# h33p/ofps

Hardware: AMD Instinct MI355X
Metric: Mvectors/s, 1080p 16x16 blocks +-16 full-search SAD (higher is better)
Workload: dtype u8

## Files before the change

ofps_amd/csrc/sad.hip:

```cpp
#include "common.hpp"

#include <cstdlib>
#include <utility>

namespace {

constexpr int kWavesPerWG = 4;

constexpr int pick_stride(int min_s, int k, int ng) {
    for (int s = min_s; s < min_s + 64; ++s)
        if ((k * s) % 32 == ng % 32) return s;
    return min_s | 1;
}

template <int B, int R, int K>
struct SadCfg {
    static_assert(B % 4 == 0 && R % 4 == 0, "tile origin must stay dword aligned");
    static_assert(B * B * 255 <= 65535, "packed u16 SAD accumulators would overflow");
    static constexpr int NCAND = 2 * R + 1;
    static constexpr int NG = (NCAND + 3) / 4;
    static constexpr int NC = (NCAND + K - 1) / K;
    static constexpr int T = NG * NC;
    static constexpr int PASSES = (T + 63) / 64;
    static constexpr int BW = B / 4;
    static constexpr int TILE_H = B + 2 * R;
    static constexpr int TILE_ROWS = NC * K + B - 1;
    static constexpr int TILE_WD = (kWavesPerWG * B + 2 * R) / 4;
    static constexpr int MAXCOL = (kWavesPerWG - 1) * BW + (NG - 1) + BW;
    static constexpr int MIN_S = (MAXCOL + 1 > TILE_WD) ? MAXCOL + 1 : TILE_WD;
    static constexpr int S = pick_stride(MIN_S, K, NG);
    static constexpr int LDS_DWORDS = TILE_ROWS * S;
};

__device__ __forceinline__ unsigned long long shfl_xor_u64(unsigned long long v, int mask) {
    unsigned lo = (unsigned)v, hi = (unsigned)(v >> 32);
    lo = __shfl_xor(lo, mask, 64);
    hi = __shfl_xor(hi, mask, 64);
    return ((unsigned long long)hi << 32) | lo;
}

struct __attribute__((packed, aligned(4))) U64A4 { unsigned long long v; };

struct SadParams {
    const uint8_t* prev_base;
    const uint8_t* cur_base;
    size_t prev_pitch, cur_pitch;
    int W, H, stride;
    int nbx, nby;
    float nx, ny;
    float4* out_entries;
    int* out_best;
    unsigned long long div_spp, div_spr;
};
inline unsigned long long div_magic48(unsigned d) { return ((1ull << 48) + d - 1) / d; }
__device__ __forceinline__ unsigned div48(unsigned n, unsigned long long m) { return (unsigned)(((unsigned long long)n * m) >> 48); }

__device__ __forceinline__ void write_block_result(const SadParams& p, int pair, int bx, int by, int B, int R,
                                                   unsigned long long key) {
    const int sad = (int)(key >> 48);
    const int dy = (int)((key >> 8) & 0xFF) - R;
    const int dx = (int)(key & 0xFF) - R;
    const size_t k = ((size_t)pair * p.nby + by) * p.nbx + bx;
    const float cx = (float)(bx * B + B / 2 + dx), cy = (float)(by * B + B / 2 + dy);
    float4 e;
    e.x = cx * p.nx;
    e.y = cy * p.ny;
    e.z = ((float)dx / 1.0f) * (-p.nx);
    e.w = ((float)dy / 1.0f) * (-p.ny);
    p.out_entries[k] = e;
    if (p.out_best) {
        p.out_best[3 * k + 0] = dx;
        p.out_best[3 * k + 1] = dy;
        p.out_best[3 * k + 2] = sad;
    }
}

template <int B, int R, int K>
__global__ __launch_bounds__(256) void sad_qsad_kernel(const SadParams p) {
    using C = SadCfg<B, R, K>;
    __shared__ uint32_t tile[C::LDS_DWORDS];

    const int pair = blockIdx.z;
    const uint8_t* __restrict__ prev = p.prev_base + (size_t)pair * p.prev_pitch;
    const uint8_t* __restrict__ cur = p.cur_base + (size_t)pair * p.cur_pitch;
    const int by = blockIdx.y;
    const int bx0 = blockIdx.x * kWavesPerWG;
    const int tid = threadIdx.x;

    const int wave = __builtin_amdgcn_readfirstlane(tid >> 6);
    const int lane = tid & 63;
    const int bx = bx0 + wave;
    const int x0 = bx * B, y0 = by * B;

    uint32_t c[B][C::BW];
    {
        const int bxc = bx < p.nbx ? bx : p.nbx - 1;
        const uint32_t* __restrict__ cp = reinterpret_cast<const uint32_t*>(cur + (size_t)y0 * p.stride + bxc * B);
        const int sdw = p.stride >> 2;
#pragma unroll
        for (int y = 0; y < B; ++y)
#pragma unroll
            for (int q = 0; q < C::BW; ++q) c[y][q] = cp[y * sdw + q];
    }

    {
        const int tx0 = bx0 * B - R, ty0 = by * B - R;
        for (int idx = tid; idx < C::TILE_H * C::TILE_WD; idx += 256) {
            const int row = idx / C::TILE_WD, col = idx - row * C::TILE_WD;
            const int gx = tx0 + 4 * col, gy = ty0 + row;
            if (gy >= 0 && gy < p.H && gx >= 0 && gx < p.W)
                tile[row * C::S + col] = *reinterpret_cast<const uint32_t*>(prev + (size_t)gy * p.stride + gx);
        }
    }
    __syncthreads();
    if (bx >= p.nbx) return;

    unsigned long long best = ~0ull;
#pragma unroll 1
    for (int pass = 0; pass < C::PASSES; ++pass) {
        const int t = pass * 64 + lane;
        const bool active = t < C::T;
        const int tc = active ? t : 0;
        const int chunk = tc / C::NG, g = tc - chunk * C::NG;
        const int dx0 = -R + 4 * g, dy0 = -R + K * chunk;

        unsigned long long acc[K];
#pragma unroll
        for (int i = 0; i < K; ++i) acc[i] = 0;

        const uint32_t* trow = tile + (K * chunk) * C::S + wave * C::BW + g;
#pragma unroll
        for (int rr = 0; rr < B + K - 1; ++rr) {
            unsigned long long win[C::BW];
#pragma unroll
            for (int q = 0; q < C::BW; ++q) win[q] = reinterpret_cast<const U64A4*>(trow + rr * C::S + q)->v;
#pragma unroll
            for (int i = 0; i < K; ++i) {
                const int y = rr - i;
                if (y >= 0 && y < B) {
#pragma unroll
                    for (int q = 0; q < C::BW; ++q) acc[i] = __builtin_amdgcn_qsad_pk_u16_u8(win[q], c[y][q], acc[i]);
                }
            }
        }
        __builtin_amdgcn_sched_group_barrier(0x100, C::BW, 0);
#pragma unroll
        for (int rr = 0; rr < B + K - 1; ++rr) {
            __builtin_amdgcn_sched_group_barrier(0x100, C::BW, 0);
            __builtin_amdgcn_sched_group_barrier(0x002, K * C::BW, 0);
        }

#pragma unroll
        for (int i = 0; i < K; ++i) asm volatile("" : "+v"(acc[i]));

        uint32_t bkey = 0xFFFFFFFFu;
        int bci = 0;
#pragma unroll
        for (int i = 0; i < K; ++i) {
            const int dy = dy0 + i;
            const int vy = (int)active & (int)(dy <= R) & (int)(y0 + dy >= 0) & (int)(y0 + dy + B <= p.H);
#pragma unroll
            for (int j = 0; j < 4; ++j) {
                const int dx = dx0 + j;
                const int v = vy & (int)(dx <= R) & (int)(x0 + dx >= 0) & (int)(x0 + dx + B <= p.W);
                const uint32_t d2inv = (uint32_t)(dx * dx + dy * dy) | (uint32_t)(v - 1);
                const uint32_t half = (j < 2) ? (uint32_t)acc[i] : (uint32_t)(acc[i] >> 32);
                const uint32_t key = ((j & 1) ? (half & 0xFFFF0000u) : (half << 16)) | d2inv;
                const bool lt = key < bkey;
                bkey = lt ? key : bkey;
                bci = lt ? (i * 4 + j) : bci;
            }
        }
        if (bkey != 0xFFFFFFFFu) {
            const int bi = bci >> 2, bj = bci & 3;
            const unsigned long long k64 =
                ((unsigned long long)bkey << 32) | (uint32_t)(((dy0 + bi + R) << 8) | (dx0 + bj + R));
            best = k64 < best ? k64 : best;
        }
    }

#pragma unroll
    for (int m = 32; m >= 1; m >>= 1) {
        const unsigned long long o = shfl_xor_u64(best, m);
        best = o < best ? o : best;
    }
    if (lane == 0) write_block_result(p, pair, bx, by, B, R, best);
}

template <int B, int R>
struct StripCfg {
    static_assert(B % 4 == 0 && R % 4 == 0, "tile origin and the dx = +R column must stay dword aligned");
    static_assert(B * B * 255 <= 65535, "packed u16 SAD accumulators would overflow");
    static constexpr int NCAND = 2 * R + 1;
    static constexpr int NGA = (2 * R) / 4;
    static constexpr int pow2_ceil(int v) { int p = 1; while (p < v) p <<= 1; return p; }
    static constexpr int NG = pow2_ceil(NGA);
    static_assert(NGA >= 1 && NG <= 64, "search range too wide for one wave per strip");
    static constexpr int NB = 64 / NG;
    static constexpr int BW = B / 4;
    static constexpr int TILE_H = B + 2 * R;
    static constexpr int KE = (NCAND + NG - 1) / NG;
    static constexpr int EDGE_COL = (2 * R) / 4;
    static constexpr int GRAN = ((NB * B) % 16 == 0 && R % 16 == 0) ? 16 : (((NB * B) % 8 == 0 && R % 8 == 0) ? 8 : 4);
    static constexpr int GDW = GRAN / 4;
    static constexpr int TILE_WG = (NB * B + 2 * R + GRAN - 1) / GRAN;
    static constexpr int MAXCOL = (NB - 1) * BW + (NG - 1) + BW;
    static constexpr int SW = ((MAXCOL + 1 > TILE_WG * GDW ? MAXCOL + 1 : TILE_WG * GDW) + 3) / 4 * 4;
    static_assert((NB - 1) * BW + EDGE_COL + BW <= SW, "edge column must lie inside a window row");
    static constexpr int TILE_ROWS = TILE_H > NG * KE + B - 1 ? TILE_H : NG * KE + B - 1;
    static constexpr int TILE_DWORDS = TILE_ROWS * SW;
    static_assert(2 * R * R < 65536, "lane key holds d2 in 16 bits");
    static constexpr int SPLIT = (NCAND + 32) / 33;
    static constexpr int NP = (NCAND + SPLIT - 1) / SPLIT;
    static constexpr int MIN_WAVES = (2 * NP + B * BW + 40 <= 168) ? 3 : 2;
    static constexpr bool COMPACT_KEY = ((2 * R * R) << 6) + NCAND < 65536 && NCAND <= 64;
    static constexpr bool RANK_KEY = !COMPACT_KEY && ((2 * R * R) << 3) + 7 < 65536;
    static constexpr int KSHIFT = COMPACT_KEY ? 6 : (RANK_KEY ? 3 : 0);
};

template <int B, int R>
struct StripWalk {
    static constexpr int ROWS_PER_BASE = (255 - StripCfg<B, R>::BW) / StripCfg<B, R>::SW + 1;
};

template <int B, int R, int I0, int RR>
__device__ __forceinline__ void strip_row(unsigned long long (&acc)[StripCfg<B, R>::NP], const uint32_t (&c)[B][B / 4],
                                          const uint32_t* lds, uint32_t& base) {
    using C = StripCfg<B, R>;
    constexpr int G = StripWalk<B, R>::ROWS_PER_BASE;
    if constexpr (RR > 0 && RR % G == 0) {
        base += G * C::SW;
        asm volatile("" : "+v"(base));
    }
    unsigned long long win[C::BW];
#pragma unroll
    for (int q = 0; q < C::BW; ++q) win[q] = reinterpret_cast<const U64A4*>(lds + base + (RR % G) * C::SW + q)->v;
#pragma unroll
    for (int ii = 0; ii < C::NP; ++ii) {
        const int y = RR - ii;
        if (I0 + ii < C::NCAND && y >= 0 && y < B) {
#pragma unroll
            for (int q = 0; q < C::BW; ++q) acc[ii] = __builtin_amdgcn_qsad_pk_u16_u8(win[q], c[y][q], acc[ii]);
        }
    }
}

template <int B, int R, int I0, int... RR>
__device__ __forceinline__ void strip_rows(unsigned long long (&acc)[StripCfg<B, R>::NP], const uint32_t (&c)[B][B / 4],
                                           const uint32_t* lds, uint32_t tile_off, std::integer_sequence<int, RR...>) {
    uint32_t base = tile_off + I0 * StripCfg<B, R>::SW;
    asm volatile("" : "+v"(base));
    (strip_row<B, R, I0, RR>(acc, c, lds, base), ...);
}

#ifndef OFPS_SAD_COLKEYS
#define OFPS_SAD_COLKEYS 2
#endif
constexpr int kSadColKeys = OFPS_SAD_COLKEYS;
constexpr int kColSlotDwords = kSadColKeys == 2 ? 4 * 64 : 0;

template <int B, int R, int I0>
__device__ __forceinline__ void strip_pass(const uint32_t (&c)[B][B / 4], const uint32_t* lds, uint32_t tile_off,
                                           const uint32_t (&colk)[4], const uint32_t (&colk_pos)[4], int y0, int H, uint32_t& bkey, int& bi,
                                           uint32_t (&colmin)[4], uint32_t* amin) {
    using C = StripCfg<B, R>;
    unsigned long long acc[C::NP];
#pragma unroll
    for (int ii = 0; ii < C::NP; ++ii) acc[ii] = 0;
    constexpr int ROWS = ((I0 + C::NP < C::NCAND ? C::NP : C::NCAND - I0) + B - 1);
    strip_rows<B, R, I0>(acc, c, lds, tile_off, std::make_integer_sequence<int, ROWS>{});
#pragma unroll
    for (int ii = 0; ii < C::NP; ++ii) asm volatile("" : "+v"(acc[ii]));
    if constexpr (kSadColKeys != 0 && (C::RANK_KEY || C::COMPACT_KEY)) {
        auto low_of = [&](int ii) -> uint32_t {
            const int i = I0 + ii, dy = -R + i;
            const bool ok = i < C::NCAND && y0 + dy >= 0 && y0 + dy + B <= H;
            return ok ? (uint32_t)(C::RANK_KEY ? ((dy * dy) << 1 | (dy > 0 ? 1 : 0)) : ((dy * dy) << 6 | i)) : 0xFFFFFFFFu;
        };
        uint32_t hmask = 0xFFFF0000u;
        asm volatile("" : "+v"(hmask));
        auto keys_of = [&](int ii, uint32_t low, uint32_t (&k)[4]) {
            const uint32_t lo = (uint32_t)acc[ii], hi = (uint32_t)(acc[ii] >> 32);
            k[0] = (lo << 16) | low; k[1] = (lo & hmask) | low; k[2] = (hi << 16) | low; k[3] = (hi & hmask) | low;
        };
        if constexpr (kSadColKeys == 1) {
#pragma unroll
            for (int ii = 0; ii < C::NP; ii += 2) {
                if (I0 + ii >= C::NCAND) break;
                uint32_t ka[4], kb[4];
                keys_of(ii, low_of(ii), ka);
                if (ii + 1 < C::NP && I0 + ii + 1 < C::NCAND) {
                    keys_of(ii + 1, low_of(ii + 1), kb);
#pragma unroll
                    for (int j = 0; j < 4; ++j)
                        asm("v_min3_u32 %0, %1, %2, %3" : "=v"(colmin[j]) : "v"(colmin[j]), "v"(ka[j]), "v"(kb[j]));
                } else {
#pragma unroll
                    for (int j = 0; j < 4; ++j) colmin[j] = min(colmin[j], ka[j]);
                }
            }
        } else {
#pragma unroll
            for (int ii = 0; ii < C::NP; ++ii) {
                if (I0 + ii >= C::NCAND) break;
                uint32_t k[4];
                keys_of(ii, low_of(ii), k);
#pragma unroll
                for (int j = 0; j < 4; ++j) __hip_atomic_fetch_min(amin + 64 * j, k[j], __ATOMIC_RELAXED, __HIP_MEMORY_SCOPE_WAVEFRONT);
            }
        }
        return;
    }
#pragma unroll
    for (int ii = 0; ii < C::NP; ++ii) {
        const int i = I0 + ii;
        const int dy = -R + i;
        if (i < C::NCAND && y0 + dy >= 0 && y0 + dy + B <= H) {
            const uint32_t lo = (uint32_t)acc[ii], hi = (uint32_t)(acc[ii] >> 32);
            const uint32_t (&ck)[4] = (C::RANK_KEY && dy > 0) ? colk_pos : colk;
            const uint32_t k0 = (lo << 16) | ck[0];
            const uint32_t k1 = (lo & 0xFFFF0000u) | ck[1];
            const uint32_t k2 = (hi << 16) | ck[2];
            const uint32_t k3 = (hi & 0xFFFF0000u) | ck[3];
            if constexpr (C::RANK_KEY) {
                bkey = min(bkey, __builtin_elementwise_add_sat(min(min(k0, k1), min(k2, k3)), (uint32_t)((dy * dy) << 3)));
            } else if constexpr (C::COMPACT_KEY) {
                const uint32_t m = __builtin_elementwise_add_sat(min(min(k0, k1), min(k2, k3)), (uint32_t)((dy * dy) << 6 | i));
                bkey = min(bkey, m);
            } else {
                const uint32_t m = __builtin_elementwise_add_sat(min(min(k0, k1), min(k2, k3)), (uint32_t)(dy * dy));
                const bool lt = m < bkey;
                bkey = lt ? m : bkey;
                bi = lt ? i : bi;
            }
        }
    }
}

template <int B, int R, int... S>
__device__ __forceinline__ void strip_passes(const uint32_t (&c)[B][B / 4], const uint32_t* lds, uint32_t tile_off,
                                             const uint32_t (&colk)[4], const uint32_t (&colk_pos)[4], int y0, int H, uint32_t& bkey, int& bi,
                                             uint32_t (&colmin)[4], uint32_t* amin, std::integer_sequence<int, S...>) {
    (strip_pass<B, R, S * StripCfg<B, R>::NP>(c, lds, tile_off, colk, colk_pos, y0, H, bkey, bi, colmin, amin), ...);
}

constexpr int kStripWaves = 4;

template <int B, int R>
__device__ __forceinline__ void strip_body(const SadParams& p, int strips_per_row, int strip, uint32_t* tiles, int wave, int lane) {
    using C = StripCfg<B, R>;
    const int strips_per_pair = strips_per_row * p.nby;
    const int pair = (int)div48((unsigned)strip, p.div_spp);
    const int rem = strip - pair * strips_per_pair;
    const int by = (int)div48((unsigned)rem, p.div_spr);
    const int bx0 = (rem - by * strips_per_row) * C::NB;

    const uint8_t* __restrict__ prev = p.prev_base + (size_t)pair * p.prev_pitch;
    const uint8_t* __restrict__ cur = p.cur_base + (size_t)pair * p.cur_pitch;
    uint32_t* tile = tiles + wave * C::TILE_DWORDS;

    const int b = lane / C::NG;
    const int g = lane % C::NG;
    const int bx = bx0 + b;
    const bool blk_on = bx < p.nbx;
    const int y0 = by * B;

    uint32_t c[B][C::BW];
    {
        const int bxc = blk_on ? bx : p.nbx - 1;
        const uint8_t* cp = cur + (size_t)y0 * p.stride + bxc * B;
#pragma unroll
        for (int y = 0; y < B; ++y) {
            if constexpr (C::BW % 4 == 0) {
#pragma unroll
                for (int q4 = 0; q4 < C::BW; q4 += 4) {
                    const uint4 v = *reinterpret_cast<const uint4*>(cp + (size_t)y * p.stride + 4 * q4);
                    c[y][q4 + 0] = v.x; c[y][q4 + 1] = v.y; c[y][q4 + 2] = v.z; c[y][q4 + 3] = v.w;
                }
            } else {
#pragma unroll
                for (int q2 = 0; q2 < C::BW; q2 += 2) {
                    const uint2 v = *reinterpret_cast<const uint2*>(cp + (size_t)y * p.stride + 4 * q2);
                    c[y][q2 + 0] = v.x; c[y][q2 + 1] = v.y;
                }
            }
        }
    }

    {
        constexpr int LR = 64 / C::TILE_WG;
        constexpr int STEPS = (C::TILE_H + LR - 1) / LR;
        const int tx0 = bx0 * B - R, ty0 = y0 - R;
        const int sr = lane / C::TILE_WG, sc = lane - sr * C::TILE_WG;
        const int gx = tx0 + C::GRAN * sc;
        const bool lane_on = sr < LR && gx >= 0 && gx < p.W;
        const uint8_t* src = prev + (ptrdiff_t)(ty0 + sr) * p.stride + gx;
        uint32_t* dst = tile + sr * C::SW + C::GDW * sc;
#pragma unroll
        for (int it = 0; it < STEPS; ++it) {
            const int row = sr + it * LR;
            const bool row_in_tile = (it + 1) * LR <= C::TILE_H || row < C::TILE_H;
            if (lane_on && row_in_tile && (unsigned)(ty0 + row) < (unsigned)p.H) {
                const uint8_t* sp = src + (ptrdiff_t)(it * LR) * p.stride;
                uint32_t* dp = dst + it * LR * C::SW;
                if constexpr (C::GRAN == 16) *reinterpret_cast<uint4*>(dp) = *reinterpret_cast<const uint4*>(sp);
                else if constexpr (C::GRAN == 8) *reinterpret_cast<uint2*>(dp) = *reinterpret_cast<const uint2*>(sp);
                else *dp = *reinterpret_cast<const uint32_t*>(sp);
            }
        }
    }
    __builtin_amdgcn_fence(__ATOMIC_RELEASE, "wavefront");
    __builtin_amdgcn_wave_barrier();
    __builtin_amdgcn_fence(__ATOMIC_ACQUIRE, "wavefront");

    const int dx0 = -R + 4 * g;
    uint32_t colk[4], colk_pos[4];
#pragma unroll
    for (int j = 0; j < 4; ++j) {
        const int dx = dx0 + j;
        const int x = bx * B + dx;
        const bool v = blk_on && g < C::NGA && x >= 0 && x + B <= p.W;
        const uint32_t rank = dx0 < 0 ? 3u - j : (uint32_t)j;
        colk[j] = v ? ((uint32_t)(dx * dx) << C::KSHIFT) | (C::RANK_KEY ? rank : 0u) : 0xFFFFFFFFu;
        colk_pos[j] = v ? ((uint32_t)(dx * dx) << C::KSHIFT) | (7u - rank) : 0xFFFFFFFFu;
    }
    uint32_t bkey = 0xFFFFFFFFu;
    int bi = 0;
    uint32_t colmin[4] = {0xFFFFFFFFu, 0xFFFFFFFFu, 0xFFFFFFFFu, 0xFFFFFFFFu};
    uint32_t* amin = nullptr;
    if constexpr (kSadColKeys == 2 && (C::RANK_KEY || C::COMPACT_KEY)) {
        amin = tiles + kStripWaves * C::TILE_DWORDS + wave * kColSlotDwords + lane;
#pragma unroll
        for (int j = 0; j < 4; ++j) amin[64 * j] = 0xFFFFFFFFu;
    }
    strip_passes<B, R>(c, tiles, (uint32_t)(wave * C::TILE_DWORDS + b * C::BW + g), colk, colk_pos, y0, p.H, bkey, bi, colmin, amin,
                       std::make_integer_sequence<int, C::SPLIT>{});
    if constexpr (kSadColKeys != 0 && (C::RANK_KEY || C::COMPACT_KEY)) {
#pragma unroll
        for (int j = 0; j < 4; ++j) {
            uint32_t kc;
            if constexpr (kSadColKeys == 2) kc = __hip_atomic_load(amin + 64 * j, __ATOMIC_RELAXED, __HIP_MEMORY_SCOPE_WAVEFRONT);
            else kc = colmin[j];
            uint32_t lk;
            if constexpr (C::RANK_KEY) {
                const uint32_t x = (((kc & 0xFFFEu) << 2) + colk[j]) ^ ((kc & 1u) * 7u);
                lk = (kc & 0xFFFF0000u) | x;
            } else {
                lk = (kc & 0xFFFF0000u) | ((kc & 0xFFFFu) + colk[j]);
            }
            lk = (colk[j] == 0xFFFFFFFFu || kc == 0xFFFFFFFFu) ? 0xFFFFFFFFu : lk;
            bkey = min(bkey, lk);
        }
    }
    unsigned long long best = ~0ull;
    if (bkey != 0xFFFFFFFFu) {
        const uint32_t d2 = (bkey & 0xFFFFu) >> C::KSHIFT;
        int dx = dx0, dy;
        if constexpr (C::RANK_KEY) {
            const int code = (int)(bkey & 7u);
            const bool neg = code < 4;
            const int rank = neg ? code : 7 - code;
            dx = dx0 + (dx0 < 0 ? 3 - rank : rank);
            const int ady = (int)(__builtin_sqrtf((float)((int)d2 - dx * dx)) + 0.5f);
            dy = neg ? -ady : ady;
        } else {
            if constexpr (C::COMPACT_KEY) bi = (int)(bkey & 63u);
            dy = -R + bi;
            const int dxsq = (int)d2 - dy * dy;
#pragma unroll
            for (int j = 1; j < 4; ++j) dx = ((dx0 + j) * (dx0 + j) == dxsq) ? dx0 + j : dx;
        }
        best = ((unsigned long long)((bkey & 0xFFFF0000u) | d2) << 32) | (unsigned long long)(uint32_t)(((dy + R) << 8) | (dx + R));
    }
    uint32_t eacc[C::KE];
#pragma unroll
    for (int i = 0; i < C::KE; ++i) eacc[i] = 0;
    {
        const uint32_t* ecol = tile + b * C::BW + C::EDGE_COL;
        const int erow0 = g * C::KE;
        uint32_t nxt[C::BW];
#pragma unroll
        for (int q = 0; q < C::BW; ++q) nxt[q] = ecol[erow0 * C::SW + q];
#pragma unroll
        for (int rr = 0; rr < B + C::KE - 1; ++rr) {
            uint32_t ref[C::BW];
#pragma unroll
            for (int q = 0; q < C::BW; ++q) ref[q] = nxt[q];
            if (rr + 1 < B + C::KE - 1) {
                const int row = erow0 + rr + 1;
#pragma unroll
                for (int q = 0; q < C::BW; ++q) nxt[q] = ecol[row * C::SW + q];
            }
#pragma unroll
            for (int i = 0; i < C::KE; ++i) {
                const int y = rr - i;
                if (y >= 0 && y < B) {
#pragma unroll
                    for (int q = 0; q < C::BW; ++q) eacc[i] = __builtin_amdgcn_sad_u8(ref[q], c[y][q], eacc[i]);
                }
            }
            asm volatile("" : "+v"(eacc[0]) : : "memory");
        }
    }

    {
        const bool xok = blk_on && bx * B + R + B <= p.W;
#pragma unroll
        for (int i = 0; i < C::KE; ++i) {
            const int dy = -R + g * C::KE + i;
            const bool v = xok && dy <= R && y0 + dy >= 0 && y0 + dy + B <= p.H;
            const unsigned long long k64 =
                ((unsigned long long)((eacc[i] << 16) | (uint32_t)(R * R + dy * dy)) << 32) |
                (unsigned long long)(uint32_t)(((dy + R) << 8) | (2 * R));
            best = (v && k64 < best) ? k64 : best;
        }
    }
#pragma unroll
    for (int m = 1; m < C::NG; m <<= 1) {
        const unsigned long long o = shfl_xor_u64(best, m);
        best = o < best ? o : best;
    }
    if (blk_on && g == 0) {
        const int sad = (int)(best >> 48);
        const int dy = (int)((best >> 8) & 0xFF) - R, dx = (int)(best & 0xFF) - R;
        const size_t k = ((size_t)pair * p.nby + by) * p.nbx + bx;
        float4 e;
        e.x = (float)(bx * B + B / 2 + dx) * p.nx;
        e.y = (float)(y0 + B / 2 + dy) * p.ny;
        e.z = ((float)dx / 1.0f) * (-p.nx);
        e.w = ((float)dy / 1.0f) * (-p.ny);
        p.out_entries[k] = e;
        if (p.out_best) {
            p.out_best[3 * k + 0] = dx;
            p.out_best[3 * k + 1] = dy;
            p.out_best[3 * k + 2] = sad;
        }
    }
}

template <int B, int R>
__global__ __launch_bounds__(64 * kStripWaves, (StripCfg<B, R>::MIN_WAVES)) void sad_strip_kernel(const SadParams p, int strips_per_row,
                                                                      int total_strips) {
    using C = StripCfg<B, R>;
    __shared__ __attribute__((aligned(16))) uint32_t tiles[kStripWaves * (C::TILE_DWORDS + kColSlotDwords)];
    const int wave = __builtin_amdgcn_readfirstlane(threadIdx.x >> 6);
    const int lane = threadIdx.x & 63;
    const int per_xcd = gridDim.x / 8;
    const int lwg = (int)(blockIdx.x % 8) * per_xcd + (int)(blockIdx.x / 8);
    const int strip = lwg * kStripWaves + wave;
    if (strip >= total_strips) return;
    strip_body<B, R>(p, strips_per_row, strip, tiles, wave, lane);
}

template <int B, int R>
__global__ __launch_bounds__(64 * kStripWaves, (StripCfg<B, R>::MIN_WAVES)) void sad_strip_list_kernel(const SadParams p, int strips_per_row,
                                                                           const uint32_t* __restrict__ strip_list) {
    using C = StripCfg<B, R>;
    __shared__ __attribute__((aligned(16))) uint32_t tiles[kStripWaves * (C::TILE_DWORDS + kColSlotDwords)];
    const int wave = __builtin_amdgcn_readfirstlane(threadIdx.x >> 6);
    const int lane = threadIdx.x & 63;
    const int count = (int)strip_list[0];
#pragma unroll 1
    for (int k = (int)blockIdx.x * kStripWaves + wave; k < count; k += (int)gridDim.x * kStripWaves)
        strip_body<B, R>(p, strips_per_row, (int)strip_list[1 + k], tiles, wave, lane);
}

struct PdeCfg {
    static constexpr int B = 16, R = 16, STEP = 4, PR = B / STEP;
    using C = StripCfg<B, R>;
    static constexpr int CUR_DW = B * C::NB * C::BW;
    static constexpr int CAP = 512;
    static constexpr int WAVE_DW = C::TILE_DWORDS + 4 + CUR_DW + CAP + 2 * C::NB;
    static constexpr int OFF_CUR = C::TILE_DWORDS + 4, OFF_LIST = OFF_CUR + CUR_DW, OFF_BEST = OFF_LIST + CAP;
    static_assert(OFF_BEST % 2 == 0, "64-bit keys must be 8-byte aligned");
};

template <int RR>
__device__ __forceinline__ void pde_row(unsigned long long (&acc)[PdeCfg::C::NP], const uint32_t (&c)[PdeCfg::PR][PdeCfg::C::BW],
                                        const uint32_t* lds, uint32_t& base) {
    using C = PdeCfg::C;
    constexpr int B = PdeCfg::B, R = PdeCfg::R, STEP = PdeCfg::STEP;
    constexpr int G = StripWalk<B, R>::ROWS_PER_BASE;
    if constexpr (RR > 0 && RR % G == 0) {
        base += G * C::SW;
        asm volatile("" : "+v"(base));
    }
    unsigned long long win[C::BW];
#pragma unroll
    for (int q = 0; q < C::BW; ++q) win[q] = reinterpret_cast<const U64A4*>(lds + base + (RR % G) * C::SW + q)->v;
#pragma unroll
    for (int ii = 0; ii < C::NP; ++ii) {
        const int y = RR - ii;
        if (ii < C::NCAND && y >= 0 && y < B && y % STEP == 0) {
#pragma unroll
            for (int q = 0; q < C::BW; ++q) acc[ii] = __builtin_amdgcn_qsad_pk_u16_u8(win[q], c[y / STEP][q], acc[ii]);
        }
    }
}
template <int... RR>
__device__ __forceinline__ void pde_rows(unsigned long long (&acc)[PdeCfg::C::NP], const uint32_t (&c)[PdeCfg::PR][PdeCfg::C::BW],
                                         const uint32_t* lds, uint32_t tile_off, std::integer_sequence<int, RR...>) {
    uint32_t base = tile_off;
    asm volatile("" : "+v"(base));
    (pde_row<RR>(acc, c, lds, base), ...);
}

__device__ __forceinline__ uint32_t pde_two_rows(const uint32_t* tile, const uint32_t* curl, int bb, int dyi, int dxi, int r8) {
    using C = PdeCfg::C;
    const int sh = dxi & 3;
    uint32_t s = 0;
#pragma unroll
    for (int k = 0; k < 2; ++k) {
        const int y = 2 * r8 + k;
        const uint32_t* rp = tile + (dyi + y) * C::SW + bb * C::BW + (dxi >> 2);
        const uint32_t* cp = curl + y * (C::NB * C::BW) + bb * C::BW;
        uint32_t d[C::BW + 1];
#pragma unroll
        for (int q = 0; q <= C::BW; ++q) d[q] = rp[q];
#pragma unroll
        for (int q = 0; q < C::BW; ++q) s = __builtin_amdgcn_sad_u8(__builtin_amdgcn_alignbyte(d[q + 1], d[q], sh), cp[q], s);
    }
    return s;
}

__global__ __launch_bounds__(64 * kStripWaves, 3) void sad_pde_kernel(const SadParams p, int strips_per_row, int total_strips,
                                                                       uint32_t* __restrict__ strip_list) {
    using P = PdeCfg;
    using C = P::C;
    constexpr int B = P::B, R = P::R;
    __shared__ __attribute__((aligned(16))) uint32_t lds[kStripWaves * P::WAVE_DW];

    const int wave = __builtin_amdgcn_readfirstlane(threadIdx.x >> 6);
    const int lane = threadIdx.x & 63;
    const int per_xcd = gridDim.x / 8;
    const int lwg = (int)(blockIdx.x % 8) * per_xcd + (int)(blockIdx.x / 8);
    const int strip = lwg * kStripWaves + wave;
    if (strip >= total_strips) return;
    const int strips_per_pair = strips_per_row * p.nby;
    const int pair = strip / strips_per_pair;
    const int rem = strip - pair * strips_per_pair;
    const int by = rem / strips_per_row;
    const int bx0 = (rem - by * strips_per_row) * C::NB;
    const uint8_t* __restrict__ prev = p.prev_base + (size_t)pair * p.prev_pitch;
    const uint8_t* __restrict__ cur = p.cur_base + (size_t)pair * p.cur_pitch;
    uint32_t* tile = lds + wave * P::WAVE_DW;
    uint32_t* curl = tile + P::OFF_CUR;
    uint32_t* list = tile + P::OFF_LIST;
    unsigned long long* bestk = reinterpret_cast<unsigned long long*>(tile + P::OFF_BEST);

    const int b = lane / C::NG, g = lane % C::NG;
    const int bx = bx0 + b;
    const bool blk_on = bx < p.nbx;
    const int y0 = by * B;

    {
        const int tx0 = bx0 * B - R, ty0 = y0 - R;
        for (int idx = lane; idx < C::TILE_H * C::TILE_WG; idx += 64) {
            const int row = idx / C::TILE_WG, col = idx - row * C::TILE_WG;
            const int gx = tx0 + 16 * col, gy = ty0 + row;
            if (gy >= 0 && gy < p.H && gx >= 0 && gx < p.W)
                *reinterpret_cast<uint4*>(tile + row * C::SW + 4 * col) = *reinterpret_cast<const uint4*>(prev + (size_t)gy * p.stride + gx);
        }
#pragma unroll
        for (int k = 0; k < 2; ++k) {
            const int idx = lane + 64 * k, row = idx / C::NB, blk = idx % C::NB;
            const int bxc = min(bx0 + blk, p.nbx - 1);
            *reinterpret_cast<uint4*>(curl + row * (C::NB * C::BW) + blk * C::BW) =
                *reinterpret_cast<const uint4*>(cur + (size_t)(y0 + row) * p.stride + bxc * B);
        }
    }
    __builtin_amdgcn_fence(__ATOMIC_RELEASE, "wavefront");
    __builtin_amdgcn_wave_barrier();
    __builtin_amdgcn_fence(__ATOMIC_ACQUIRE, "wavefront");

    uint32_t c4[P::PR][C::BW];
#pragma unroll
    for (int r = 0; r < P::PR; ++r)
#pragma unroll
        for (int q = 0; q < C::BW; ++q) c4[r][q] = curl[(P::STEP * r) * (C::NB * C::BW) + b * C::BW + q];
    unsigned long long acc[C::NP];
#pragma unroll
    for (int ii = 0; ii < C::NP; ++ii) acc[ii] = 0;
    pde_rows(acc, c4, lds, (uint32_t)(wave * P::WAVE_DW + b * C::BW + g), std::make_integer_sequence<int, C::NCAND + B - 1>{});
#pragma unroll
    for (int ii = 0; ii < C::NP; ++ii) asm volatile("" : "+v"(acc[ii]));

    const int dx0 = -R + 4 * g;
    bool colv[4];
    uint32_t colk[4];
#pragma unroll
    for (int j = 0; j < 4; ++j) {
        const int x = bx * B + dx0 + j;
        colv[j] = blk_on && x >= 0 && x + B <= p.W;
        colk[j] = colv[j] ? (uint32_t)((dx0 + j) * (dx0 + j)) << C::KSHIFT : 0xFFFFFFFFu;
    }
    static_assert(C::COMPACT_KEY && C::SPLIT == 1, "written for the +-16 geometry");
    uint32_t bkey = 0xFFFFFFFFu;
#pragma unroll
    for (int i = 0; i < C::NCAND; ++i) {
        const int dy = -R + i;
        if (y0 + dy >= 0 && y0 + dy + B <= p.H) {
            const uint32_t lo = (uint32_t)acc[i], hi = (uint32_t)(acc[i] >> 32);
            const uint32_t k0 = (lo << 16) | colk[0], k1 = (lo & 0xFFFF0000u) | colk[1];
            const uint32_t k2 = (hi << 16) | colk[2], k3 = (hi & 0xFFFF0000u) | colk[3];
            bkey = min(bkey, __builtin_elementwise_add_sat(min(min(k0, k1), min(k2, k3)), (uint32_t)((dy * dy) << 6 | i)));
        }
    }
    unsigned long long pbest = ~0ull;
    if (bkey != 0xFFFFFFFFu) {
        const int bi = (int)(bkey & 63u), dy = -R + bi;
        const uint32_t d2 = (bkey & 0xFFFFu) >> C::KSHIFT;
        const int dxsq = (int)d2 - dy * dy;
        int dx = dx0;
#pragma unroll
        for (int j = 1; j < 4; ++j) dx = ((dx0 + j) * (dx0 + j) == dxsq) ? dx0 + j : dx;
        pbest = ((unsigned long long)((bkey & 0xFFFF0000u) | d2) << 32) | (unsigned long long)(uint32_t)(((dy + R) << 8) | (dx + R));
    }
    uint32_t eacc[C::KE];
    const bool xok = blk_on && bx * B + R + B <= p.W;
    {
        const uint32_t* ecol = tile + b * C::BW + C::EDGE_COL;
#pragma unroll
        for (int i = 0; i < C::KE; ++i) {
            const int dyi = min(g * C::KE + i, C::NCAND - 1);
            uint32_t sacc = 0;
#pragma unroll
            for (int r = 0; r < P::PR; ++r)
#pragma unroll
                for (int q = 0; q < C::BW; ++q) sacc = __builtin_amdgcn_sad_u8(ecol[(dyi + P::STEP * r) * C::SW + q], c4[r][q], sacc);
            eacc[i] = sacc;
            const int dy = -R + g * C::KE + i;
            const bool v = xok && dy <= R && y0 + dy >= 0 && y0 + dy + B <= p.H;
            const unsigned long long k64 = ((unsigned long long)((sacc << 16) | (uint32_t)(R * R + dy * dy)) << 32) |
                                           (unsigned long long)(uint32_t)(((dy + R) << 8) | (2 * R));
            pbest = (v && k64 < pbest) ? k64 : pbest;
        }
    }
#pragma unroll
    for (int m = 1; m < C::NG; m <<= 1) {
        const unsigned long long o = shfl_xor_u64(pbest, m);
        pbest = o < pbest ? o : pbest;
    }
    const int dy0i = blk_on ? (int)((pbest >> 8) & 0xFF) : R, dx0i = blk_on ? (int)(pbest & 0xFF) : R;
    auto key64 = [&](uint32_t sad, int dyi, int dxi) {
        const int dy = dyi - R, dx = dxi - R;
        return ((unsigned long long)((sad << 16) | (uint32_t)(dx * dx + dy * dy)) << 32) | (unsigned long long)(uint32_t)((dyi << 8) | dxi);
    };
    uint32_t U = pde_two_rows(tile, curl, b, dy0i, dx0i, g);
#pragma unroll
    for (int m = 1; m < C::NG; m <<= 1) U += __shfl_xor(U, m, 64);
    if (g == 0) bestk[b] = blk_on ? key64(U, dy0i, dx0i) : ~0ull;
    int nlist = 0;
    {
        int uj[4];
#pragma unroll
        for (int j = 0; j < 4; ++j) uj[j] = colv[j] ? (int)U : -1;
        const unsigned long long below = (1ull << lane) - 1ull;
        typedef unsigned short us2 __attribute__((ext_vector_type(2)));
        const uint32_t u1 = min(U + 1u, 0xFFFFu) * 0x10001u;
        auto any_le = [&](uint32_t v) {
            const us2 m = __builtin_elementwise_min(__builtin_bit_cast(us2, v), __builtin_bit_cast(us2, u1));
            return __builtin_bit_cast(uint32_t, m) ^ u1;
        };
#pragma unroll
        for (int i = 0; i < C::NCAND; ++i) {
            const int dy = -R + i;
            if (y0 + dy >= 0 && y0 + dy + B <= p.H) {
                const uint32_t lo = (uint32_t)acc[i], hi = (uint32_t)(acc[i] >> 32);
                if (!__ballot((any_le(lo) | any_le(hi)) != 0u)) continue;
                const int s4[4] = {(int)(lo & 0xFFFFu), (int)(lo >> 16), (int)(hi & 0xFFFFu), (int)(hi >> 16)};
#pragma unroll
                for (int j = 0; j < 4; ++j) {
                    const bool hit = s4[j] <= uj[j];
                    const unsigned long long mask = __ballot(hit);
                    if (mask) {
                        const int pos = nlist + __popcll(mask & below);
                        if (hit && pos < P::CAP) list[pos] = ((uint32_t)b << 16) | ((uint32_t)i << 8) | (uint32_t)(4 * g + j);
                        nlist += __popcll(mask);
                    }
                }
            }
        }
#pragma unroll
        for (int i = 0; i < C::KE; ++i) {
            const int dyi = g * C::KE + i, dy = dyi - R;
            const bool hit = xok && dy <= R && y0 + dy >= 0 && y0 + dy + B <= p.H && eacc[i] <= U;
            const unsigned long long mask = __ballot(hit);
            if (mask) {
                const int pos = nlist + __popcll(mask & below);
                if (hit && pos < P::CAP) list[pos] = ((uint32_t)b << 16) | ((uint32_t)dyi << 8) | (uint32_t)(2 * R);
                nlist += __popcll(mask);
            }
        }
    }
    __builtin_amdgcn_fence(__ATOMIC_RELEASE, "wavefront");
    __builtin_amdgcn_wave_barrier();
    __builtin_amdgcn_fence(__ATOMIC_ACQUIRE, "wavefront");
    const int n = nlist;
    if (n > P::CAP) {
        if (lane == 0) {
            const uint32_t pos = atomicAdd(&strip_list[0], 1u);
            strip_list[1 + pos] = (uint32_t)strip;
        }
        return;
    }
    constexpr int PER_STEP = 2 * (64 / C::NG);
    for (int base = 0; base < n; base += PER_STEP) {
        const int idx0 = base + lane / C::NG, idx1 = idx0 + 64 / C::NG;
        const uint32_t e0 = list[min(idx0, n - 1)], e1 = list[min(idx1, n - 1)];
        const int bb0 = (int)(e0 >> 16), dyi0 = (int)((e0 >> 8) & 0xFF), dxi0 = (int)(e0 & 0xFF);
        const int bb1 = (int)(e1 >> 16), dyi1 = (int)((e1 >> 8) & 0xFF), dxi1 = (int)(e1 & 0xFF);
        uint32_t s0 = pde_two_rows(tile, curl, bb0, dyi0, dxi0, g);
        uint32_t s1 = pde_two_rows(tile, curl, bb1, dyi1, dxi1, g);
#pragma unroll
        for (int m = 1; m < C::NG; m <<= 1) { s0 += __shfl_xor(s0, m, 64); s1 += __shfl_xor(s1, m, 64); }
        if (g == 0 && idx0 < n) atomicMin(&bestk[bb0], key64(s0, dyi0, dxi0));
        if (g == 0 && idx1 < n) atomicMin(&bestk[bb1], key64(s1, dyi1, dxi1));
    }
// ... 296 lines not shown
```

Before: 516.6.

## Clip vertical candidate rows at frame edges and split edge-column SAD work

At blocks near the top or bottom frame edges, a clipped strip path runs only the 8-row candidate chunks that overlap the valid dy range, skipping SAD work for out-of-frame displacements. The dx=+R edge column now spreads 2R rows across lanes. The last dy=+R candidate is computed by a cross-lane partial sum over block rows, using current-block rows loaded straight from global memory. This also raises the minimum-waves hint for the 8x8/R=8 config. The cost is more code paths, extra global loads and a shuffle reduction.

```diff
diff --git a/ofps_amd/csrc/sad.hip b/ofps_amd/csrc/sad.hip
--- a/ofps_amd/csrc/sad.hip
+++ b/ofps_amd/csrc/sad.hip
@@ -200,6 +200,8 @@
     static constexpr int BW = B / 4;
     static constexpr int TILE_H = B + 2 * R;
     static constexpr int KE = (NCAND + NG - 1) / NG;
+    static constexpr int KE2 = (2 * R + NG - 1) / NG;
+    static constexpr int ERL = (B + NG - 1) / NG;
     static constexpr int EDGE_COL = (2 * R) / 4;
     static constexpr int GRAN = ((NB * B) % 16 == 0 && R % 16 == 0) ? 16 : (((NB * B) % 8 == 0 && R % 8 == 0) ? 8 : 4);
     static constexpr int GDW = GRAN / 4;
@@ -212,7 +214,7 @@
     static_assert(2 * R * R < 65536, "lane key holds d2 in 16 bits");
     static constexpr int SPLIT = (NCAND + 32) / 33;
     static constexpr int NP = (NCAND + SPLIT - 1) / SPLIT;
-    static constexpr int MIN_WAVES = (2 * NP + B * BW + 40 <= 168) ? 3 : 2;
+    static constexpr int MIN_WAVES = (B == 8 && R == 8) ? 8 : ((2 * NP + B * BW + 40 <= 168) ? 3 : 2);
     static constexpr bool COMPACT_KEY = ((2 * R * R) << 6) + NCAND < 65536 && NCAND <= 64;
     static constexpr bool RANK_KEY = !COMPACT_KEY && ((2 * R * R) << 3) + 7 < 65536;
     static constexpr int KSHIFT = COMPACT_KEY ? 6 : (RANK_KEY ? 3 : 0);
@@ -223,8 +225,8 @@
     static constexpr int ROWS_PER_BASE = (255 - StripCfg<B, R>::BW) / StripCfg<B, R>::SW + 1;
 };
 
-template <int B, int R, int I0, int RR>
-__device__ __forceinline__ void strip_row(unsigned long long (&acc)[StripCfg<B, R>::NP], const uint32_t (&c)[B][B / 4],
+template <int B, int R, int I0, int N, int RR>
+__device__ __forceinline__ void strip_row(unsigned long long (&acc)[N], const uint32_t (&c)[B][B / 4],
                                           const uint32_t* lds, uint32_t& base) {
     using C = StripCfg<B, R>;
     constexpr int G = StripWalk<B, R>::ROWS_PER_BASE;
@@ -236,7 +238,7 @@
 #pragma unroll
     for (int q = 0; q < C::BW; ++q) win[q] = reinterpret_cast<const U64A4*>(lds + base + (RR % G) * C::SW + q)->v;
 #pragma unroll
-    for (int ii = 0; ii < C::NP; ++ii) {
+    for (int ii = 0; ii < N; ++ii) {
         const int y = RR - ii;
         if (I0 + ii < C::NCAND && y >= 0 && y < B) {
 #pragma unroll
@@ -245,12 +247,12 @@
     }
 }
 
-template <int B, int R, int I0, int... RR>
-__device__ __forceinline__ void strip_rows(unsigned long long (&acc)[StripCfg<B, R>::NP], const uint32_t (&c)[B][B / 4],
+template <int B, int R, int I0, int N, int... RR>
+__device__ __forceinline__ void strip_rows(unsigned long long (&acc)[N], const uint32_t (&c)[B][B / 4],
                                            const uint32_t* lds, uint32_t tile_off, std::integer_sequence<int, RR...>) {
     uint32_t base = tile_off + I0 * StripCfg<B, R>::SW;
     asm volatile("" : "+v"(base));
-    (strip_row<B, R, I0, RR>(acc, c, lds, base), ...);
+    (strip_row<B, R, I0, N, RR>(acc, c, lds, base), ...);
 }
 
 #ifndef OFPS_SAD_COLKEYS
@@ -259,18 +261,18 @@
 constexpr int kSadColKeys = OFPS_SAD_COLKEYS;
 constexpr int kColSlotDwords = kSadColKeys == 2 ? 4 * 64 : 0;
 
-template <int B, int R, int I0>
+template <int B, int R, int I0, int N = StripCfg<B, R>::NP>
 __device__ __forceinline__ void strip_pass(const uint32_t (&c)[B][B / 4], const uint32_t* lds, uint32_t tile_off,
                                            const uint32_t (&colk)[4], const uint32_t (&colk_pos)[4], int y0, int H, uint32_t& bkey, int& bi,
                                            uint32_t (&colmin)[4], uint32_t* amin) {
     using C = StripCfg<B, R>;
-    unsigned long long acc[C::NP];
-#pragma unroll
-    for (int ii = 0; ii < C::NP; ++ii) acc[ii] = 0;
-    constexpr int ROWS = ((I0 + C::NP < C::NCAND ? C::NP : C::NCAND - I0) + B - 1);
-    strip_rows<B, R, I0>(acc, c, lds, tile_off, std::make_integer_sequence<int, ROWS>{});
-#pragma unroll
-    for (int ii = 0; ii < C::NP; ++ii) asm volatile("" : "+v"(acc[ii]));
+    unsigned long long acc[N];
+#pragma unroll
+    for (int ii = 0; ii < N; ++ii) acc[ii] = 0;
+    constexpr int ROWS = ((I0 + N < C::NCAND ? N : C::NCAND - I0) + B - 1);
+    strip_rows<B, R, I0, N>(acc, c, lds, tile_off, std::make_integer_sequence<int, ROWS>{});
+#pragma unroll
+    for (int ii = 0; ii < N; ++ii) asm volatile("" : "+v"(acc[ii]));
     if constexpr (kSadColKeys != 0 && (C::RANK_KEY || C::COMPACT_KEY)) {
         auto low_of = [&](int ii) -> uint32_t {
             const int i = I0 + ii, dy = -R + i;
@@ -285,11 +287,11 @@
         };
         if constexpr (kSadColKeys == 1) {
 #pragma unroll
-            for (int ii = 0; ii < C::NP; ii += 2) {
+            for (int ii = 0; ii < N; ii += 2) {
                 if (I0 + ii >= C::NCAND) break;
                 uint32_t ka[4], kb[4];
                 keys_of(ii, low_of(ii), ka);
-                if (ii + 1 < C::NP && I0 + ii + 1 < C::NCAND) {
+                if (ii + 1 < N && I0 + ii + 1 < C::NCAND) {
                     keys_of(ii + 1, low_of(ii + 1), kb);
 #pragma unroll
                     for (int j = 0; j < 4; ++j)
@@ -301,7 +303,7 @@
             }
         } else {
 #pragma unroll
-            for (int ii = 0; ii < C::NP; ++ii) {
+            for (int ii = 0; ii < N; ++ii) {
                 if (I0 + ii >= C::NCAND) break;
                 uint32_t k[4];
                 keys_of(ii, low_of(ii), k);
@@ -312,7 +314,7 @@
         return;
     }
 #pragma unroll
-    for (int ii = 0; ii < C::NP; ++ii) {
+    for (int ii = 0; ii < N; ++ii) {
         const int i = I0 + ii;
         const int dy = -R + i;
         if (i < C::NCAND && y0 + dy >= 0 && y0 + dy + B <= H) {
@@ -344,6 +346,24 @@
     (strip_pass<B, R, S * StripCfg<B, R>::NP>(c, lds, tile_off, colk, colk_pos, y0, H, bkey, bi, colmin, amin), ...);
 }
 
+template <int B, int R>
+struct StripClip {
+    static constexpr int NCH = (2 * R) / 8 > 0 ? (2 * R) / 8 : 1;
+    static constexpr int start(int k) { return k >= NCH ? StripCfg<B, R>::NCAND : (8 * k > R ? 8 * k + 1 : 8 * k); }
+};
+
+template <int B, int R, int... K>
+__device__ __forceinline__ void strip_clipped(const uint32_t (&c)[B][B / 4], const uint32_t* lds, uint32_t tile_off,
+                                              const uint32_t (&colk)[4], const uint32_t (&colk_pos)[4], int y0, int H, int ilo, int ihi,
+                                              uint32_t& bkey, int& bi, uint32_t (&colmin)[4], uint32_t* amin, std::integer_sequence<int, K...>) {
+    using L = StripClip<B, R>;
+    auto chunk = [&](auto k) {
+        constexpr int S = L::start(decltype(k)::value), E = L::start(decltype(k)::value + 1);
+        if (ihi >= S && ilo < E) strip_pass<B, R, S, E - S>(c, lds, tile_off, colk, colk_pos, y0, H, bkey, bi, colmin, amin);
+    };
+    (chunk(std::integral_constant<int, K>{}), ...);
+}
+
 constexpr int kStripWaves = 4;
 
 template <int B, int R>
@@ -433,8 +453,14 @@
 #pragma unroll
         for (int j = 0; j < 4; ++j) amin[64 * j] = 0xFFFFFFFFu;
     }
-    strip_passes<B, R>(c, tiles, (uint32_t)(wave * C::TILE_DWORDS + b * C::BW + g), colk, colk_pos, y0, p.H, bkey, bi, colmin, amin,
-                       std::make_integer_sequence<int, C::SPLIT>{});
+    const int ilo = __builtin_amdgcn_readfirstlane(R - y0 > 0 ? R - y0 : 0);
+    const int ihi = __builtin_amdgcn_readfirstlane(p.H - B - y0 < R ? R + p.H - B - y0 : 2 * R);
+    const uint32_t lane_off = (uint32_t)(wave * C::TILE_DWORDS + b * C::BW + g);
+    if (ilo == 0 && ihi == 2 * R)
+        strip_passes<B, R>(c, tiles, lane_off, colk, colk_pos, y0, p.H, bkey, bi, colmin, amin, std::make_integer_sequence<int, C::SPLIT>{});
+    else
+        strip_clipped<B, R>(c, tiles, lane_off, colk, colk_pos, y0, p.H, ilo, ihi, bkey, bi, colmin, amin,
+                            std::make_integer_sequence<int, StripClip<B, R>::NCH>{});
     if constexpr (kSadColKeys != 0 && (C::RANK_KEY || C::COMPACT_KEY)) {
 #pragma unroll
         for (int j = 0; j < 4; ++j) {
@@ -472,27 +498,52 @@
         }
         best = ((unsigned long long)((bkey & 0xFFFF0000u) | d2) << 32) | (unsigned long long)(uint32_t)(((dy + R) << 8) | (dx + R));
     }
-    uint32_t eacc[C::KE];
-#pragma unroll
-    for (int i = 0; i < C::KE; ++i) eacc[i] = 0;
+    uint32_t eacc[C::KE2];
+#pragma unroll
+    for (int i = 0; i < C::KE2; ++i) eacc[i] = 0;
+    uint32_t elast = 0;
+    const uint32_t* ecol = tile + b * C::BW + C::EDGE_COL;
     {
-        const uint32_t* ecol = tile + b * C::BW + C::EDGE_COL;
-        const int erow0 = g * C::KE;
+        const int yl = g * C::ERL;
+        uint32_t cl[C::ERL][C::BW];
+        {
+            const int bxc = blk_on ? bx : p.nbx - 1;
+            const uint8_t* cp = cur + (size_t)y0 * p.stride + bxc * B;
+#pragma unroll
+            for (int r = 0; r < C::ERL; ++r) {
+                const int y = (C::NG * C::ERL > B && yl + r > B - 1) ? B - 1 : yl + r;
+                const uint8_t* rp = cp + (size_t)y * p.stride;
+                if constexpr (C::BW % 4 == 0) {
+#pragma unroll
+                    for (int q4 = 0; q4 < C::BW; q4 += 4) {
+                        const uint4 v = *reinterpret_cast<const uint4*>(rp + 4 * q4);
+                        cl[r][q4 + 0] = v.x; cl[r][q4 + 1] = v.y; cl[r][q4 + 2] = v.z; cl[r][q4 + 3] = v.w;
+                    }
+                } else {
+#pragma unroll
+                    for (int q2 = 0; q2 < C::BW; q2 += 2) {
+                        const uint2 v = *reinterpret_cast<const uint2*>(rp + 4 * q2);
+                        cl[r][q2 + 0] = v.x; cl[r][q2 + 1] = v.y;
+                    }
+                }
+            }
+        }
+        const int erow0 = g * C::KE2;
         uint32_t nxt[C::BW];
 #pragma unroll
         for (int q = 0; q < C::BW; ++q) nxt[q] = ecol[erow0 * C::SW + q];
 #pragma unroll
-        for (int rr = 0; rr < B + C::KE - 1; ++rr) {
+        for (int rr = 0; rr < B + C::KE2 - 1; ++rr) {
             uint32_t ref[C::BW];
 #pragma unroll
             for (int q = 0; q < C::BW; ++q) ref[q] = nxt[q];
-            if (rr + 1 < B + C::KE - 1) {
+            if (rr + 1 < B + C::KE2 - 1) {
                 const int row = erow0 + rr + 1;
 #pragma unroll
                 for (int q = 0; q < C::BW; ++q) nxt[q] = ecol[row * C::SW + q];
             }
 #pragma unroll
-            for (int i = 0; i < C::KE; ++i) {
+            for (int i = 0; i < C::KE2; ++i) {
                 const int y = rr - i;
                 if (y >= 0 && y < B) {
 #pragma unroll
@@ -501,19 +552,41 @@
             }
             asm volatile("" : "+v"(eacc[0]) : : "memory");
         }
+#pragma unroll
+        for (int i = 1; i < C::KE2; ++i) asm volatile("" : "+v"(eacc[i]));
+#pragma unroll
+        for (int r = 0; r < C::ERL; ++r) {
+            const int y = (C::NG * C::ERL > B && yl + r > B - 1) ? B - 1 : yl + r;
+#pragma unroll
+            for (int q = 0; q < C::BW; ++q) elast = __builtin_amdgcn_sad_u8(ecol[(2 * R + y) * C::SW + q], cl[r][q], elast);
+        }
+        if constexpr (C::NG * C::ERL > B) elast = yl < B ? elast : 0u;
+#pragma unroll
+        for (int m = 1; m < C::NG; m <<= 1) elast += (uint32_t)__shfl_xor((int)elast, m, 64);
     }
 
     {
         const bool xok = blk_on && bx * B + R + B <= p.W;
-#pragma unroll
-        for (int i = 0; i < C::KE; ++i) {
-            const int dy = -R + g * C::KE + i;
-            const bool v = xok && dy <= R && y0 + dy >= 0 && y0 + dy + B <= p.H;
-            const unsigned long long k64 =
-                ((unsigned long long)((eacc[i] << 16) | (uint32_t)(R * R + dy * dy)) << 32) |
-                (unsigned long long)(uint32_t)(((dy + R) << 8) | (2 * R));
-            best = (v && k64 < best) ? k64 : best;
-        }
+        const int chi = ihi < 2 * R - 1 ? ihi : 2 * R - 1;
+        uint32_t ek = 0xFFFFFFFFu;
+        int ei = 0;
+#pragma unroll
+        for (int i = 0; i < C::KE2; ++i) {
+            const int idx = g * C::KE2 + i, dy = idx - R;
+            const bool v = (unsigned)(idx - ilo) <= (unsigned)(chi - ilo);
+            const uint32_t k = v ? ((eacc[i] << 16) | (uint32_t)(R * R + dy * dy)) : 0xFFFFFFFFu;
+            const bool lt = k < ek;
+            ek = lt ? k : ek;
+            ei = lt ? idx : ei;
+        }
+        if (ihi == 2 * R) {
+            const uint32_t k = (elast << 16) | (uint32_t)(2 * R * R);
+            const bool lt = k < ek;
+            ek = lt ? k : ek;
+            ei = lt ? 2 * R : ei;
+        }
+        const unsigned long long k64 = ((unsigned long long)ek << 32) | (unsigned long long)(uint32_t)((ei << 8) | (2 * R));
+        best = (xok && ek != 0xFFFFFFFFu && k64 < best) ? k64 : best;
     }
 #pragma unroll
     for (int m = 1; m < C::NG; m <<= 1) {
```

Measured after the change: 526.9, median of 6. 2.0% higher.
